# Gadersd/stable-diffusion-xl-burn

Hardware: NVIDIA H100
Metric: unet_sampler_steps_per_sec_1024x1024_bs1 (higher is better)
Workload: dtype f16

## Files before the change

### stable-diffusion-xl-burn_b200/csrc/common.cuh

```cuda
#pragma once
#include <cuda_fp16.h>
#include <cuda_runtime.h>
#include <stdint.h>
#include <stdio.h>

namespace sdxl {

__device__ __forceinline__ uint32_t smem_u32(const void* p) {
  return static_cast<uint32_t>(__cvta_generic_to_shared(p));
}
__device__ __forceinline__ float warp_sum(float v) {
#pragma unroll
  for (int o = 16; o > 0; o >>= 1) v += __shfl_xor_sync(0xffffffffu, v, o);
  return v;
}
__device__ __forceinline__ float warp_max(float v) {
#pragma unroll
  for (int o = 16; o > 0; o >>= 1) v = fmaxf(v, __shfl_xor_sync(0xffffffffu, v, o));
  return v;
}
__device__ __forceinline__ float silu_f(float x) { return x / (1.0f + __expf(-x)); }
__device__ __forceinline__ float erf_as(float x) {
  const float ax = fabsf(x);
  float t;
// ... 37 lines not shown
__device__ __forceinline__ void mbar_arrive(uint64_t* bar) {
  asm volatile("mbarrier.arrive.shared::cta.b64 _, [%0];" ::"r"(smem_u32(bar)) : "memory");
}
__device__ __forceinline__ bool mbar_try_wait(uint64_t* bar, uint32_t parity) {
  uint32_t ok;
  asm volatile(
      "{\n\t"
      ".reg .pred p;\n\t"
      "mbarrier.try_wait.parity.shared::cta.b64 p, [%1], %2;\n\t"
      "selp.u32 %0, 1, 0, p;\n\t"
      "}"
      : "=r"(ok)
      : "r"(smem_u32(bar)), "r"(parity)
      : "memory");
  return ok != 0;
}
__device__ __forceinline__ void mbar_wait(uint64_t* bar, uint32_t parity) {
  if (mbar_try_wait(bar, parity)) return;
  const uint64_t t0 = globaltimer_ns();
  while (!mbar_try_wait(bar, parity)) {
    if (globaltimer_ns() - t0 > 4000000000ull) {
      printf("sdxl_b200: mbarrier wait timeout (block %d,%d,%d thread %d)\n", blockIdx.x, blockIdx.y,
             blockIdx.z, threadIdx.x);
      __trap();
    }
  }
}
__device__ __forceinline__ void mbar_wait_nocall(uint64_t* bar, uint32_t parity) {
  if (mbar_try_wait(bar, parity)) return;
  const uint64_t t0 = globaltimer_ns();
  while (!mbar_try_wait(bar, parity))
    if (globaltimer_ns() - t0 > 4000000000ull) __trap();
}
__device__ __forceinline__ void fence_proxy_async_smem() {
  asm volatile("fence.proxy.async.shared::cta;" ::: "memory");
}

__device__ __forceinline__ void tma_prefetch_desc(const void* tmap) {
  asm volatile("prefetch.tensormap [%0];" ::"l"(reinterpret_cast<uint64_t>(tmap)) : "memory");
}
__device__ __forceinline__ void tma_load_2d(void* dst, const void* tmap, uint64_t* bar, int c0, int c1) {
  asm volatile(
      "cp.async.bulk.tensor.2d.shared::cluster.global.mbarrier::complete_tx::bytes [%0], [%1, {%3, %4}], [%2];"
      ::"r"(smem_u32(dst)), "l"(reinterpret_cast<uint64_t>(tmap)), "r"(smem_u32(bar)), "r"(c0), "r"(c1)
      : "memory");
}
__device__ __forceinline__ void tma_load_3d(void* dst, const void* tmap, uint64_t* bar, int c0, int c1,
                                            int c2) {
  asm volatile(
      "cp.async.bulk.tensor.3d.shared::cluster.global.mbarrier::complete_tx::bytes [%0], [%1, {%3, %4, %5}], [%2];"
      ::"r"(smem_u32(dst)), "l"(reinterpret_cast<uint64_t>(tmap)), "r"(smem_u32(bar)), "r"(c0), "r"(c1),
      "r"(c2)
      : "memory");
}
__device__ __forceinline__ void tma_load_4d(void* dst, const void* tmap, uint64_t* bar, int c0, int c1,
                                            int c2, int c3) {
  asm volatile(
      "cp.async.bulk.tensor.4d.shared::cluster.global.mbarrier::complete_tx::bytes [%0], [%1, {%3, %4, %5, %6}], [%2];"
      ::"r"(smem_u32(dst)), "l"(reinterpret_cast<uint64_t>(tmap)), "r"(smem_u32(bar)), "r"(c0), "r"(c1),
      "r"(c2), "r"(c3)
      : "memory");
}

__device__ __forceinline__ void wg_fence() { asm volatile("wgmma.fence.sync.aligned;" ::: "memory"); }
__device__ __forceinline__ void wg_commit() { asm volatile("wgmma.commit_group.sync.aligned;" ::: "memory"); }
template <int N>
__device__ __forceinline__ void wg_wait() {
  asm volatile("wgmma.wait_group.sync.aligned %0;" ::"n"(N) : "memory");
}
__device__ __forceinline__ uint64_t wg_desc_sw128(uint32_t saddr) {
  const uint32_t lo = ((saddr >> 4) & 0x3FFFu) | (1u << 16);
  const uint32_t hi = 64u  | (1u << 30) ;
  return (static_cast<uint64_t>(hi) << 32) | lo;
}
__device__ __forceinline__ void wgmma_ss_n160(float (&d)[80], uint64_t da, uint64_t db, int scale_d) {
  asm volatile(
      "{\n\t.reg .pred p;\n\tsetp.ne.b32 p, %82, 0;\n\t"
// ... 28 lines not shown
```

### stable-diffusion-xl-burn_b200/csrc/engine_core.h

```cpp
#pragma once
#include "../../include/sdxl_b200.h"
#include "kernels.h"

#include <math.h>
#include <nvtx3/nvToolsExt.h>
#include <stdarg.h>
#include <stdio.h>
#include <stdlib.h>
#include <string.h>

#include <map>
#include <memory>
#include <string>
#include <type_traits>
#include <vector>

using namespace sdxl;

struct sdxl_ctx {
  int device = 0;
  cudaStream_t stream = nullptr;
  bool own_stream = false;
  int num_sms = 132;
  std::string err;
// ... 686 lines not shown
  for (size_t i = 0; i < n && !r; ++i) {
    r = exec_op(c, P->ops[i]);
    if (!r && cudaEventRecord(ev[i + 1], c->stream) != cudaSuccess) r = -2;
  }
  cudaError_t se = cudaStreamSynchronize(c->stream);
  ms.assign(n, 0.f);
  if (!r && se == cudaSuccess)
    for (size_t i = 0; i < n; ++i) cudaEventElapsedTime(&ms[i], ev[i], ev[i + 1]);
  for (auto& e : ev) cudaEventDestroy(e);
  if (se != cudaSuccess) return fail(c, (int)se, "profile run failed: %s", cudaGetErrorString(se));
  return r;
}

static int profile_plan_impl(sdxl_ctx* c, Plan* P, double* ms_by_kind, double* flops_by_kind, int* launches_by_kind) {
  std::vector<float> ms;
  const int r = time_plan_ops(c, P, ms);
  for (int k = 0; k < SDXL_PROFILE_KINDS; ++k) { ms_by_kind[k] = 0; flops_by_kind[k] = 0; launches_by_kind[k] = 0; }
  if (r) return r;
  for (size_t i = 0; i < ms.size(); ++i) {
    const int k = (int)P->ops[i].kind;
    if (k < 0 || k >= SDXL_PROFILE_KINDS) continue;
    ms_by_kind[k] += ms[i];
    flops_by_kind[k] += P->ops[i].flops;
    launches_by_kind[k] += (P->ops[i].kind == OP_GN) ? 2 : 1;
  }
  return 0;
}

static int profile_dump_impl(sdxl_ctx* c, Plan* P, const char* path) {
  std::vector<float> ms;
  if (int r = time_plan_ops(c, P, ms)) return r;
  FILE* f = fopen(path, "w");
  if (!f) return fail(c, -3, "cannot open %s", path);
  fprintf(f, "op,kind,us,gflop,tflops,M_tiles,N,BN,Kblocks,T,S,heads\n");
  for (size_t i = 0; i < ms.size(); ++i) {
    const Op& o = P->ops[i];
    int mt = 0, N = 0, BN = 0, kb = 0, T = 0, S = 0, H = 0;
    if (o.kind == OP_IGEMM) {
      mt = o.ig.tilesW * o.ig.tilesH * o.ig.tilesB; N = o.ig.N; BN = o.ig.BN;
      for (int s2 = 0; s2 < o.ig.nseg; ++s2) kb += o.ig.seg[s2].nkb;
    } else if (o.kind == OP_ATTN) { T = o.at.T; S = o.at.S; H = o.at.n_head; }
    fprintf(f, "%zu,%s,%.2f,%.3f,%.1f,%d,%d,%d,%d,%d,%d,%d\n", i, kOpNames[o.kind], ms[i] * 1e3, o.flops * 1e-9,
            ms[i] > 0 ? o.flops / (ms[i] * 1e-3) * 1e-12 : 0.0, mt, N, BN, kb, T, S, H);
  }
  fclose(f);
  return 0;
}

struct TmpBufs {
  std::vector<void*> p;
  cudaStream_t st;
  int fill = debug_fill_byte();
  explicit TmpBufs(cudaStream_t s) : st(s) {}
  template <typename T>
  T* get(size_t bytes) {
    void* d = nullptr;
    if (cudaMallocAsync(&d, bytes ? bytes : 16, st) != cudaSuccess) return nullptr;
    p.push_back(d);
    if (fill >= 0) debug_fill((T*)d, bytes / sizeof(T), st, fill);
    return (T*)d;
  }
  ~TmpBufs() { for (void* d : p) cudaFreeAsync(d, st); }
};

static int adapters_apply(sdxl_ctx* c, AdapterState& S, int n, const sdxl_adapter* ad) {
  if (n < 0 || n > SDXL_MAX_ADAPTERS) return fail(c, 4600, "set_adapters: n = %d outside [0, %d]", n, SDXL_MAX_ADAPTERS);
  if (n > 0 && !ad) return fail(c, 4601, "set_adapters: null adapter array");
  TmpBufs tmp(c->stream);
  std::map<std::string, std::vector<LoraTerm>> terms;
  for (int a = 0; a < n; ++a) {
    PackView pv;
    std::vector<uint8_t> table;
    if (!ad[a].pack) return fail(c, 4602, "set_adapters: adapter %d has a null pack", a);
    int r = parse_pack(c, ad[a].pack, ad[a].bytes, ad[a].pack_on_device, pv, table);
    if (r) { c->err = "adapter " + std::to_string(a) + ": " + c->err; return r; }
    if (ad[a].pack_on_device) {
// ... 113 lines not shown
```

### stable-diffusion-xl-burn_b200/csrc/igemm.cu

```cuda
#include "common.cuh"
#include "kernels.h"

#include <stdio.h>
#include <stdlib.h>

namespace sdxl {

static constexpr int kTileM = 128;
static constexpr int kBlockK = 64;
static constexpr int kABytes = kTileM * kBlockK * 2;
static constexpr int kConsumerWarps = 8;
static constexpr int kThreads = 128 + kConsumerWarps * 32;

__device__ __forceinline__ size_t out_pixel(const IgemmParams& p, int tb, int th, int tw, int r, bool& ok, int& bb) {
  const int wt = r % p.Wt, ht = (r / p.Wt) % p.Ht, bt = r / (p.Wt * p.Ht);
  bb = tb * p.Bt + bt;
  const int hh = th * p.Ht + ht, ww = tw * p.Wt + wt;
  ok = (bb < p.Bn) && (hh < p.H) && (ww < p.W);
  return ok ? ((size_t)bb * p.H + hh) * (size_t)p.opix_row + (size_t)ww * p.opix_w + p.opix_off : 0;
}

__device__ __forceinline__ void store2(const IgemmParams& p, size_t off, float x0, float x1, bool two, bool vec) {
  if (p.out_f32) {
    float* o = reinterpret_cast<float*>(p.out) + off;
// ... 34 lines not shown
          bv[jj] = rv[jj] = make_float2(0.f, 0.f);
          if (n >= p.N) continue;
          if (bias) bv[jj] = (two && vec) ? __ldg(reinterpret_cast<const float2*>(bias + n)) : make_float2(bias[n], two ? bias[n + 1] : 0.f);
          if (res) rv[jj] = (two && vec) ? *reinterpret_cast<const float2*>(res + n) : make_float2(res[n], two ? res[n + 1] : 0.f);
        }
#pragma unroll
        for (int jj = 0; jj < JC; ++jj) {
          const int j = j0 + jj, n = n0 + 8 * j + cq;
          if (n >= p.N) continue;
          float x0 = acc[4 * j + 2 * h], x1 = acc[4 * j + 2 * h + 1];
          if (bias) { x0 += bv[jj].x; x1 += bv[jj].y; }
          if (res) { x0 += rv[jj].x; x1 += rv[jj].y; }
          store2(p, pix * p.ldo + n, x0, x1, n + 1 < p.N, vec);
        }
      }
    } else {
      constexpr int hb = BN / 2;
#pragma unroll
      for (int j = 0; j < hb / 8; ++j) {
        const int c = 8 * j + cq;
        float x0 = acc[4 * j + 2 * h], x1 = acc[4 * j + 2 * h + 1];
        float y0 = acc[4 * (j + hb / 8) + 2 * h], y1 = acc[4 * (j + hb / 8) + 2 * h + 1];
        if (p.bias != nullptr) {
          x0 += __ldg(p.bias + n0 + c); x1 += __ldg(p.bias + n0 + c + 1);
          y0 += __ldg(p.bias + n0 + hb + c); y1 += __ldg(p.bias + n0 + hb + c + 1);
        }
        reinterpret_cast<__half2*>(reinterpret_cast<__half*>(p.out) + pix * p.ldo + nt * hb + c)[0] =
            __floats2half2_rn(x0 * gelu_erf_f(y0), x1 * gelu_erf_f(y1));
      }
    }
  }
}

template <int BN>
__global__ void __launch_bounds__(kThreads, 1) igemm_kernel(const __grid_constant__ IgemmParams p) {
  constexpr int NC = BN == 160 ? 160 : BN >= 128 ? 128 : 64;
  constexpr int NCH = BN / NC;
  extern __shared__ __align__(1024) uint8_t smem_raw[];
  uint8_t* smem = reinterpret_cast<uint8_t*>((reinterpret_cast<uintptr_t>(smem_raw) + 1023) & ~uintptr_t(1023));
  const int nst = p.nstages;
  constexpr uint32_t stage_bytes = kABytes + BN * 128;
  uint64_t* full_bar = reinterpret_cast<uint64_t*>(smem + (size_t)nst * stage_bytes);
  uint64_t* empty_bar = full_bar + nst;

  const int warp = threadIdx.x >> 5, lane = threadIdx.x & 31;
  const int m_tiles = p.tilesW * p.tilesH * p.tilesB;
  const int num_tiles = m_tiles * p.tilesN;
  int total_kb = 0;
  for (int s = 0; s < p.nseg; ++s) total_kb += p.seg[s].nkb;

  if (threadIdx.x == 0) {
    for (int i = 0; i < nst; ++i) { mbar_init(&full_bar[i], 1); mbar_init(&empty_bar[i], kConsumerWarps); }
    fence_barrier_init();
    tma_prefetch_desc(&p.tmA0);
    tma_prefetch_desc(&p.tmA1);
    tma_prefetch_desc(&p.tmB);
  }
  __syncthreads();
  griddep_wait();
  griddep_launch_dependents();

  if (warp < 4) {
    setmaxnreg_dec<40>();
    if (warp != 0 || lane != 0) return;
    uint32_t stage = 0, phase = 0;
    for (int st = blockIdx.x; st < num_tiles; st += gridDim.x) {
      const int mt = st % m_tiles, nt = st / m_tiles;
      const int tw = mt % p.tilesW, th = (mt / p.tilesW) % p.tilesH, tb = mt / (p.tilesW * p.tilesH);
      const int w0 = tw * p.Wt, h0 = th * p.Ht, b0 = tb * p.Bt, n0 = nt * BN;
      int kcol = 0;
      for (int s = 0; s < p.nseg; ++s) {
        const IgemmSeg sg = p.seg[s];
        const void* mapA = sg.map ? (const void*)&p.tmA1 : (const void*)&p.tmA0;
        for (int j = 0; j < sg.nkb; ++j, kcol += kBlockK) {
          mbar_wait_nocall(&empty_bar[stage], phase ^ 1);
          uint8_t* dst = smem + stage * stage_bytes;
          mbar_expect_tx(&full_bar[stage], stage_bytes);
          tma_load_4d(dst, mapA, &full_bar[stage], j * kBlockK, w0 + sg.dw, h0 + sg.dh, b0 + sg.db);
          tma_load_2d(dst + kABytes, &p.tmB, &full_bar[stage], kcol, n0);
          if (++stage == (uint32_t)nst) { stage = 0; phase ^= 1; }
        }
      }
    }
    return;
  }

  setmaxnreg_inc<232>();
  const int wg = (warp >> 2) - 1;
  const int r0 = wg * 64 + (warp & 3) * 16 + (lane >> 2);
  const uint32_t smem_base = smem_u32(smem);
  uint32_t stage = 0, phase = 0;
  float acc[BN / 2];
  for (int st = blockIdx.x; st < num_tiles; st += gridDim.x) {
    const int mt = st % m_tiles, nt = st / m_tiles;
    uint32_t prev = 0;
    for (int kb = 0; kb < total_kb; ++kb) {
      mbar_wait_nocall(&full_bar[stage], phase);
      wg_fence();
      const uint32_t a = smem_base + stage * stage_bytes + (uint32_t)wg * (64 * 128);
      const uint32_t b = smem_base + stage * stage_bytes + kABytes;
#pragma unroll
      for (int k = 0; k < kBlockK / 16; ++k) {
        const uint64_t da = wg_desc_sw128(a + 32 * k);
#pragma unroll
        for (int c = 0; c < NCH; ++c) {
          const uint64_t db = wg_desc_sw128(b + c * NC * 128 + 32 * k);
          if constexpr (NC == 160) wgmma_ss_n160(*reinterpret_cast<float(*)[80]>(acc), da, db, (kb | k) != 0);
          else if constexpr (NC == 128) wgmma_ss_n128(*reinterpret_cast<float(*)[64]>(acc + 64 * c), da, db, (kb | k) != 0);
          else wgmma_ss_n64(*reinterpret_cast<float(*)[32]>(acc + 32 * c), da, db, (kb | k) != 0);
        }
      }
      wg_commit();
      if (kb > 0) {
        wg_wait<1>();
        if (lane == 0) mbar_arrive(&empty_bar[prev]);
      }
      prev = stage;
      if (++stage == (uint32_t)nst) { stage = 0; phase ^= 1; }
    }
    wg_wait<0>();
    if (lane == 0 && total_kb > 0) mbar_arrive(&empty_bar[prev]);
    const int tw = mt % p.tilesW, th = (mt / p.tilesW) % p.tilesH, tb = mt / (p.tilesW * p.tilesH);
    epilogue<BN>(p, acc, tb, th, tw, nt, r0, lane);
  }
}

typedef CUresult (*PFN_encodeTiled)(CUtensorMap*, CUtensorMapDataType, cuuint32_t, void*, const cuuint64_t*,
                                    const cuuint64_t*, const cuuint32_t*, const cuuint32_t*,
                                    CUtensorMapInterleave, CUtensorMapSwizzle, CUtensorMapL2promotion,
                                    CUtensorMapFloatOOBfill);
static PFN_encodeTiled get_encode() {
  static PFN_encodeTiled fn = nullptr;
  if (!fn) {
    void* f = nullptr;
    cudaDriverEntryPointQueryResult qres;
    if (cudaGetDriverEntryPoint("cuTensorMapEncodeTiled", &f, cudaEnableDefault, &qres) != cudaSuccess ||
        qres != cudaDriverEntryPointSuccess)
      return nullptr;
    fn = reinterpret_cast<PFN_encodeTiled>(f);
  }
  return fn;
}

static int encode(CUtensorMap* tm, const void* base, int rank, const uint64_t* dims, const uint64_t* strides_bytes,
                  const uint32_t* box, CUtensorMapDataType dtype = CU_TENSOR_MAP_DATA_TYPE_FLOAT16,
                  CUtensorMapSwizzle swz = CU_TENSOR_MAP_SWIZZLE_128B) {
  PFN_encodeTiled fn = get_encode();
  if (!fn) return 1001;
  cuuint64_t gd[5];
  cuuint64_t gs[5];
  cuuint32_t bx[5], es[5];
  for (int i = 0; i < rank; ++i) {
    gd[i] = dims[i];
    bx[i] = box[i];
    es[i] = 1;
    if (i > 0) gs[i - 1] = strides_bytes[i - 1];
// ... 29 lines not shown
  uint64_t str[2] = {(uint64_t)pitch * 2, (uint64_t)rows_per_batch * pitch * 2};
  uint32_t box[3] = {64, 128, 1};
  return encode(tm, base, 3, dims, str, box);
}

void igemm_pick_box(int W, int H, int* Wt, int* Ht, int* Bt) {
  int wt = 1;
  while (wt * 2 <= W && wt * 2 <= 128) wt *= 2;
  int ht = 1;
  while (ht * 2 <= H && wt * ht * 2 <= 128) ht *= 2;
  *Wt = wt;
  *Ht = ht;
  *Bt = 128 / (wt * ht);
}

int igemm_pick_bn(int m_tiles, int N, int num_sms, bool geglu) {
  (void)geglu;
  double best = 1e30;
  int best_bn = 0;
  for (int bn : {256, 160, 128, 64}) {
    if (N % bn) continue;
    const long tiles = (long)m_tiles * (N / bn);
    const long waves = (tiles + num_sms - 1) / num_sms;
    const double cost = (double)waves * (bn + 48.0);
    if (cost < best) {
      best = cost;
      best_bn = bn;
    }
  }
  if (!best_bn) best_bn = N <= 64 ? 64 : N <= 128 ? 128 : 256;
  return best_bn;
}

struct IgemmDev { bool attr = false; int num_sms = 0; };
static IgemmDev g_igemm_dev[64];
static IgemmDev* igemm_dev() {
  int dev = 0;
  if (cudaGetDevice(&dev) != cudaSuccess || dev < 0 || dev >= 64) return nullptr;
  IgemmDev& D = g_igemm_dev[dev];
  if (!D.num_sms) {
    cudaDeviceGetAttribute(&D.num_sms, cudaDevAttrMultiProcessorCount, dev);
    if (D.num_sms <= 0) D.num_sms = 132;
  }
  return &D;
}
static int device_sms() {
  IgemmDev* D = igemm_dev();
  return D ? D->num_sms : 132;
}

static constexpr int kMaxSmem = 227 * 1024;
static size_t igemm_smem_bytes(int nst, int BN) { return (size_t)nst * (kABytes + BN * 128) + 1024  + 2 * nst * 8; }

int igemm_configure(IgemmParams& p, const IgemmOperands& o, int outW, int outH, int outB, int mode, int geglu_bn) {
  igemm_pick_box(outW, outH, &p.Wt, &p.Ht, &p.Bt);
  p.W = outW; p.H = outH; p.Bn = outB;
  p.opix_row = outW; p.opix_w = 1; p.opix_off = 0;
  p.tilesW = (outW + p.Wt - 1) / p.Wt;
  p.tilesH = (outH + p.Ht - 1) / p.Ht;
  p.tilesB = (outB + p.Bt - 1) / p.Bt;
  const int m_tiles = p.tilesW * p.tilesH * p.tilesB;
  p.N = o.N;
  p.mode = mode;
  p.BN = (mode == IGEMM_GEGLU) ? geglu_bn : igemm_pick_bn(m_tiles, o.N, device_sms(), false);
  if (p.BN != 64 && p.BN != 128 && p.BN != 160 && p.BN != 256) return 1010;
  p.tilesN = (mode == IGEMM_GEGLU) ? (o.N / p.BN) : ((o.N + p.BN - 1) / p.BN);
  int r = make_tmap_act(&p.tmA0, o.a0, o.a0Bn, o.a0H, o.a0W, o.a0C, o.a0pitch, p.Wt, p.Ht, p.Bt);
  if (!r && o.a1) r = make_tmap_act(&p.tmA1, o.a1, o.a1Bn, o.a1H, o.a1W, o.a1C, o.a1pitch, p.Wt, p.Ht, p.Bt);
  if (!r && !o.a1) p.tmA1 = p.tmA0;
  if (!r) r = make_tmap_wgt(&p.tmB, o.w, o.N, o.Ktot, p.BN);
  if (r) return r;
  const int stage_bytes = kABytes + p.BN * 128;
  int nst = (kMaxSmem - 1024 - 256) / stage_bytes;
  if (nst > 8) nst = 8;
  p.nstages = nst;
  return 0;
}

int igemm_launch(cudaStream_t st, IgemmParams& p) {
  if (p.res != nullptr && p.ldr != p.ldo) return 1003;
  if ((unsigned long long)p.Bn * p.H * (unsigned long long)p.opix_row * (unsigned long long)p.ldo >= (1ull << 32)) return 1004;
  if (p.nstages < 2) return 1011;
  const size_t smem = igemm_smem_bytes(p.nstages, p.BN);
  if (smem > (size_t)kMaxSmem) return 1011;
  IgemmDev* D = igemm_dev();
  if (!D) return 1009;
  if (!D->attr) {
    cudaError_t e = cudaFuncSetAttribute(igemm_kernel<64>, cudaFuncAttributeMaxDynamicSharedMemorySize, kMaxSmem);
    if (e == cudaSuccess) e = cudaFuncSetAttribute(igemm_kernel<128>, cudaFuncAttributeMaxDynamicSharedMemorySize, kMaxSmem);
    if (e == cudaSuccess) e = cudaFuncSetAttribute(igemm_kernel<160>, cudaFuncAttributeMaxDynamicSharedMemorySize, kMaxSmem);
    if (e == cudaSuccess) e = cudaFuncSetAttribute(igemm_kernel<256>, cudaFuncAttributeMaxDynamicSharedMemorySize, kMaxSmem);
    if (e != cudaSuccess) return (int)e;
    D->attr = true;
  }
  const long tiles = (long)p.tilesW * p.tilesH * p.tilesB * p.tilesN;
  const dim3 grid((unsigned)(tiles < D->num_sms ? (tiles > 0 ? tiles : 1) : D->num_sms));
  switch (p.BN) {
    case 64: return launch_kernel(igemm_kernel<64>, grid, dim3(kThreads), smem, st, true, p);
    case 128: return launch_kernel(igemm_kernel<128>, grid, dim3(kThreads), smem, st, true, p);
    case 160: return launch_kernel(igemm_kernel<160>, grid, dim3(kThreads), smem, st, true, p);
    case 256: return launch_kernel(igemm_kernel<256>, grid, dim3(kThreads), smem, st, true, p);
    default: return 1010;
  }
}

}
```

### stable-diffusion-xl-burn_b200/csrc/kernels.h

```cpp
#pragma once
#include <cuda.h>
#include <cuda_fp16.h>
#include <cuda_runtime.h>
#include <stdint.h>

namespace sdxl {

bool pdl_enabled();
template <typename... KArgs, typename... Args>
inline int launch_kernel(void (*kernel)(KArgs...), dim3 grid, dim3 block, size_t smem, cudaStream_t st, bool pdl,
                         Args&&... args) {
  cudaLaunchConfig_t cfg{};
  cfg.gridDim = grid;
  cfg.blockDim = block;
  cfg.dynamicSmemBytes = smem;
  cfg.stream = st;
  cudaLaunchAttribute attr[1];
  attr[0].id = cudaLaunchAttributeProgrammaticStreamSerialization;
  attr[0].val.programmaticStreamSerializationAllowed = 1;
  cfg.attrs = attr;
  cfg.numAttrs = (pdl && pdl_enabled()) ? 1 : 0;
  return (int)cudaLaunchKernelEx(&cfg, kernel, static_cast<KArgs>(args)...);
}
template <typename... KArgs, typename... Args>
// ... 34 lines not shown
    if (e != cudaSuccess) return (int)e;
    done[dev] = true;
  }
  return 0;
}

constexpr int IGEMM_MAX_SEG = 20;
struct IgemmSeg {
  int16_t map;
  int16_t dw, dh;
  int16_t db;
  int32_t nkb;
};
enum IgemmMode : int { IGEMM_LINEAR = 0, IGEMM_GEGLU = 1 };
struct alignas(64) IgemmParams {
  CUtensorMap tmA0, tmA1, tmB;
  IgemmSeg seg[IGEMM_MAX_SEG];
  int nseg;
  int Wt, Ht, Bt;
  int W, H, Bn;
  int tilesW, tilesH, tilesB, tilesN;
  int N;
  int BN;
  int nstages;
  int mode;
  void* out;
  int out_f32;
  int ldo;
  const float* bias;
  int bias_bstride;
  const float* res;
  int ldr;
  int opix_row, opix_w, opix_off;
};
int make_tmap_act(CUtensorMap* tm, const __half* base, int Bn, int H, int W, int C, int pitch, int Wt,
                  int Ht, int Bt);
int make_tmap_wgt(CUtensorMap* tm, const __half* base, int N, int K, int BN);
void igemm_pick_box(int W, int H, int* Wt, int* Ht, int* Bt);
struct IgemmOperands {
  const __half* a0; int a0Bn, a0H, a0W, a0C, a0pitch;
  const __half* a1; int a1Bn, a1H, a1W, a1C, a1pitch;
  const __half* w; int N, Ktot;
};
int igemm_configure(IgemmParams& p, const IgemmOperands& o, int outW, int outH, int outB, int mode, int geglu_bn);
int igemm_launch(cudaStream_t st, IgemmParams& p);
int igemm_pick_bn(int m_tiles, int N, int num_sms, bool geglu);

constexpr int ATTN_MAX_SRC = 8;
struct AttnIpSource {
  CUtensorMap tm;
  int S, k_col0, v_col0;
  const float* scale;
  const float* mask;
};
struct AttnParams {
  CUtensorMap tmQ, tmK, tmV;
  int T, S, n_head, B;
  int q_col0, k_col0, v_col0;
  __half* out;
  int ldo;
  float scale_log2e;
  CUtensorMap tmKip, tmVip;
  int S_ip;
  int k_ip_col0, v_ip_col0;
  const float* ip_scale;
  int n_src;
  const float* ip_mask;
  AttnIpSource ip_src[ATTN_MAX_SRC - 1];
};
int make_tmap_rows(CUtensorMap* tm, const __half* base, int rows_per_batch, int nbatch, int cols, int pitch);
int attention_launch(cudaStream_t st, const AttnParams& p);
int ip_mask_resize_launch(cudaStream_t st, const float* mask, int H, int W, int mh, int mw, int T, float* out);

struct GnParams {
  const float* x1; int C1;
  const float* x2; int C2;
  int B, HW, n_group;
  const float* gamma; const float* beta;
// ... 121 lines not shown
```

### stable-diffusion-xl-burn_b200/csrc/testing.cu

```cuda
#include "kernels.h"
#include "schedule.h"

#define SDXL_TEST_API extern "C" __attribute__((visibility("default")))

using namespace sdxl;

SDXL_TEST_API int sdxl_test_igemm(void* stream, const void* a0, int a0Bn, int a0H, int a0W, int a0C, int a0pitch, const void* a1,
                                  int a1Bn, int a1H, int a1W, int a1C, int a1pitch, const void* w, int N, int Ktot, int outW,
                                  int outH, int outB, int mode, int geglu_bn, const int* segs, int nseg, void* out, int out_f32,
                                  int ldo, const float* bias, int bias_bstride, const float* res, int ldr, int opix_row,
                                  int opix_w, int opix_off) {
  if (nseg < 1 || nseg > IGEMM_MAX_SEG) return 5002;
  IgemmParams p{};
  p.nseg = nseg;
  for (int i = 0; i < nseg; ++i)
    p.seg[i] = {(int16_t)segs[5 * i], (int16_t)segs[5 * i + 1], (int16_t)segs[5 * i + 2], (int16_t)segs[5 * i + 3], segs[5 * i + 4]};
  p.out = out; p.out_f32 = out_f32; p.ldo = ldo;
  p.bias = bias; p.bias_bstride = bias_bstride;
  p.res = res; p.ldr = ldr;
  const IgemmOperands o{(const __half*)a0, a0Bn, a0H, a0W, a0C, a0pitch, (const __half*)a1, a1Bn, a1H, a1W, a1C, a1pitch,
                        (const __half*)w, N, Ktot};
  if (int r = igemm_configure(p, o, outW, outH, outB, mode, geglu_bn)) return r;
  if (opix_row) { p.opix_row = opix_row; p.opix_w = opix_w; p.opix_off = opix_off; }
  return igemm_launch((cudaStream_t)stream, p);
}

SDXL_TEST_API int sdxl_test_attention(void* stream, const void* q, int q_pitch, int q_col0, const void* kv, int kv_pitch, int k_col0,
                                      int v_col0, int B, int T, int S, int n_head, void* out, int ldo, const void* kip,
                                      int kip_pitch, int k_ip_col0, int v_ip_col0, int S_ip, const float* ip_scale) {
  AttnParams p{};
  p.T = T; p.S = S; p.n_head = n_head; p.B = B;
  p.q_col0 = q_col0; p.k_col0 = k_col0; p.v_col0 = v_col0;
  p.out = (__half*)out; p.ldo = ldo;
  p.scale_log2e = (float)(1.4426950408889634 / 8.0);
  int r = make_tmap_rows(&p.tmQ, (const __half*)q, T, B, q_pitch, q_pitch);
  if (!r) r = make_tmap_rows(&p.tmK, (const __half*)kv, S, B, kv_pitch, kv_pitch);
  if (r) return r;
  p.tmV = p.tmK;
  if (kip) {
    p.S_ip = S_ip; p.k_ip_col0 = k_ip_col0; p.v_ip_col0 = v_ip_col0; p.ip_scale = ip_scale; p.n_src = 1;
    if ((r = make_tmap_rows(&p.tmKip, (const __half*)kip, S_ip, B, kip_pitch, kip_pitch))) return r;
    p.tmVip = p.tmKip;
  }
  return attention_launch((cudaStream_t)stream, p);
}

SDXL_TEST_API int sdxl_test_attention_multi(void* stream, const void* q, int q_pitch, int q_col0, const void* kv, int kv_pitch, int k_col0,
                                            int v_col0, int B, int T, int S, int n_head, void* out, int ldo, int n_src,
                                            const void* const* src_kv, const int* src_info, const float* const* scales,
                                            const float* const* masks) {
  if (n_src < 1 || n_src > ATTN_MAX_SRC) return 5003;
  AttnParams p{};
  p.T = T; p.S = S; p.n_head = n_head; p.B = B;
  p.q_col0 = q_col0; p.k_col0 = k_col0; p.v_col0 = v_col0;
  p.out = (__half*)out; p.ldo = ldo;
  p.scale_log2e = (float)(1.4426950408889634 / 8.0);
// ... 227 lines not shown
```

### stable-diffusion-xl-burn_b200/sdxl_b200/_testing.py

```python
from __future__ import annotations

import ctypes as C
import os
from typing import Optional, Sequence

import torch

from ._lib import SdxlError, SdxlLibraryMissing

HERE = os.path.dirname(os.path.abspath(__file__))
LIB_PATH = os.path.join(HERE, "libsdxl_b200_testing.so")

P, I, F, L, Z = C.c_void_p, C.c_int, C.c_float, C.c_long, C.c_size_t
PROTOTYPES = {
    "sdxl_test_igemm": (I, [P, P, I, I, I, I, I, P, I, I, I, I, I, P, I, I, I, I, I, I, I, P, I, P, I, I, P, I, P, I, I, I, I]),
    "sdxl_test_attention": (I, [P, P, I, I, P, I, I, I, I, I, I, I, P, I, P, I, I, I, I, P]),
    "sdxl_test_attention_multi": (I, [P, P, I, I, P, I, I, I, I, I, I, I, P, I, I, P, P, P, P]),
    "sdxl_test_ip_mask_resize": (I, [P, P, I, I, I, I, I, P]),
    "sdxl_test_attention_small": (I, [P, P, I, I, P, P, I, I, I, I, I, I, I, P, I, P, I, I]),
    "sdxl_test_perceiver_ln": (I, [P, P, P, I, I, I, I, P, P, P, P, F, P, P]),
    "sdxl_test_gn_scratch_floats": (C.c_size_t, [I, I]),
    "sdxl_test_gn_scratch_init": (I, [P, P, I, I]),
    "sdxl_test_gn": (I, [P, P, I, P, I, I, I, I, P, P, F, I, P, P, P, P]),
    "sdxl_test_gemv": (I, [P, P, I, I, I, P, I, P, P, I, I, I, I, P, I]),
    "sdxl_test_conv_in": (I, [P, P, I, I, I, I, I, I, P, P, I, P, P, I]),
    "sdxl_test_conv_in_cat": (I, [P, P, I, I, I, I, P, I, I, I, I, P, P, I, P]),
    "sdxl_test_pag_identity": (I, [P, P, I, C.c_long, P]),
    "sdxl_test_cfg_pag_ddim": (I, [P, P, I, I, I, I, I, F, F, F, F, F, F, P]),
    "sdxl_test_freeu_twiddles": (None, [I, I, P]),
    "sdxl_test_freeu": (I, [P, P, I, P, I, I, I, I, P, P, P]),
    "sdxl_test_repack_upconv": (I, [P, P, I, I, P, I]),
    "sdxl_test_repack_conv": (I, [P, P, I, I, I, I, P, I, I, I]),
    "sdxl_test_transpose_linear": (I, [P, P, I, I, P, I, I, I]),
    "sdxl_test_bias_to_f32": (I, [P, P, I, P, I, I]),
    "sdxl_test_lora_merge": (I, [P, I, I, I, I, P, P, P, P, P, P, I, C.c_size_t, I, I, I, I, P]),
    "sdxl_test_lora_upconv_merge": (I, [P, P, P, I, I, P, I]),
    "sdxl_test_softmax_rows": (I, [P, P, Z, I, I, F, P, Z]),
    "sdxl_test_transpose_f16": (I, [P, P, Z, I, I, P, Z]),
    "sdxl_test_post_quant": (I, [P, P, I, I, I, P, P, F, P]),
    "sdxl_test_quant_out": (I, [P, P, I, I, I, L, P, P, F, P]),
    "sdxl_test_image_u8": (I, [P, P, L, I, P]),
    "sdxl_test_image_from_u8": (I, [P, P, I, L, P]),
    "sdxl_test_embed_tokens": (I, [P, P, I, I, I, I, P, P, P, P]),
    "sdxl_test_patchify": (I, [P, P, I, I, I, I, P]),
    "sdxl_test_vision_embed_ln": (I, [P, P, P, P, I, I, I, P, P, F, P]),
    "sdxl_test_mlp_act": (I, [P, P, Z, I, P]),
    "sdxl_test_ln_gather_f32": (I, [P, P, P, I, I, I, P, P, F, P]),
    "sdxl_test_pixel_unshuffle": (I, [P, P, I, I, I, I, P]),
# ... 18 lines not shown
    "sdxl_test_timestep_embedding_f32": (I, [P, P, I, I, F, P]),
}
_lib = None


def load() -> C.CDLL:
    global _lib
    if _lib is None:
        if not os.path.exists(LIB_PATH):
            raise SdxlLibraryMissing(f"{LIB_PATH} not found: build it with `python stable-diffusion-xl-burn_b200/build.py`")
        lib = C.CDLL(LIB_PATH)
        for name, (res, args) in PROTOTYPES.items():
            fn = getattr(lib, name)
            fn.restype = res
            fn.argtypes = args
        _lib = lib
    return _lib


def _p(t: Optional[torch.Tensor]):
    if t is None:
        return None
    assert t.is_cuda and t.is_contiguous(), "kernel operands are contiguous CUDA tensors"
    return t.data_ptr()


def _call(name: str, *args) -> None:
    lib = load()
    rc = getattr(lib, name)(torch.cuda.current_stream().cuda_stream, *args)
    if rc != 0:
        raise SdxlError(f"{name} failed ({rc})")


def igemm(a0: torch.Tensor, a0_shape: Sequence[int], w: torch.Tensor, N: int, Ktot: int, out_whb: Sequence[int],
          segs: Sequence[Sequence[int]], out: torch.Tensor, ldo: int, *, a1: Optional[torch.Tensor] = None,
          a1_shape: Sequence[int] = (0, 0, 0, 0), bias: Optional[torch.Tensor] = None, bias_bstride: int = 0,
          res: Optional[torch.Tensor] = None, ldr: int = 0, mode: int = 0, geglu_bn: int = 0,
          opix: Optional[Sequence[int]] = None) -> None:
    seg = (C.c_int * (5 * len(segs)))(*[int(v) for s in segs for v in s])
    o = opix or (0, 0, 0)
    _call("sdxl_test_igemm", _p(a0), *a0_shape, a0_shape[3], _p(a1), *a1_shape, a1_shape[3], _p(w), N, Ktot, *out_whb, mode,
          geglu_bn, seg, len(segs), _p(out), int(out.dtype == torch.float32), ldo, _p(bias), bias_bstride, _p(res), ldr, *o)


def attention(q: torch.Tensor, q_pitch: int, q_col0: int, kv: torch.Tensor, kv_pitch: int, k_col0: int, v_col0: int,
              B: int, T: int, S: int, n_head: int, out: torch.Tensor, ldo: int, kip: Optional[torch.Tensor] = None,
              kip_pitch: int = 0, k_ip_col0: int = 0, v_ip_col0: int = 0, S_ip: int = 0,
              ip_scale: Optional[torch.Tensor] = None) -> None:
    _call("sdxl_test_attention", _p(q), q_pitch, q_col0, _p(kv), kv_pitch, k_col0, v_col0, B, T, S, n_head, _p(out), ldo,
          _p(kip), kip_pitch, k_ip_col0, v_ip_col0, S_ip, _p(ip_scale))


def attention_multi(q: torch.Tensor, q_pitch: int, q_col0: int, kv: torch.Tensor, kv_pitch: int, k_col0: int, v_col0: int,
                    B: int, T: int, S: int, n_head: int, out: torch.Tensor, ldo: int, sources: Sequence[tuple]) -> None:
    n = len(sources)
    kvs = (C.c_void_p * n)(*[_p(s[0]) for s in sources])
    info = (C.c_int * (4 * n))(*[int(v) for s in sources for v in (s[1], s[2], s[3], s[4])])
    scales = (C.c_void_p * n)(*[_p(s[5]) for s in sources])
    masks = (C.c_void_p * n)(*[_p(s[6]) for s in sources])
    _call("sdxl_test_attention_multi", _p(q), q_pitch, q_col0, _p(kv), kv_pitch, k_col0, v_col0, B, T, S, n_head, _p(out), ldo, n,
          kvs, info, scales, masks)


def ip_mask_resize(mask: torch.Tensor, mh: int, mw: int, T: int) -> torch.Tensor:
    out = torch.empty(T, device=mask.device, dtype=torch.float32)
    _call("sdxl_test_ip_mask_resize", _p(mask), mask.shape[0], mask.shape[1], mh, mw, T, _p(out))
    return out


def attention_small(q, q_pitch, q_col0, k, v, kv_pitch, k_col0, v_col0, B, T, S, n_head, mask, causal, out, ldo,
                    head_dim) -> None:
    _call("sdxl_test_attention_small", _p(q), q_pitch, q_col0, _p(k), _p(v), kv_pitch, k_col0, v_col0, B, T, S, n_head,
          _p(mask), int(causal), _p(out), ldo, head_dim)


# ... 202 lines not shown
```

Before: 27.34.

## Add 2-CTA cluster mode with TMA multicast of weight tiles in igemm

Adds a cluster-of-2 variant of the implicit-GEMM kernel in which paired CTAs along M each load half of the shared B (weight) tile and multicast it to both CTAs. Empty barriers now count arrivals from both CTAs so a stage is refilled only once both consumers have released it. Auto policy enables clusters only when tiles fit in one wave and M tiles are even, aiming to halve weight-load traffic for small-grid GEMMs. Risks include extra cross-CTA synchronization, cluster scheduling limits, and a drain loop at producer exit.

```diff
diff --git a/stable-diffusion-xl-burn_b200/csrc/common.cuh b/stable-diffusion-xl-burn_b200/csrc/common.cuh
--- a/stable-diffusion-xl-burn_b200/csrc/common.cuh
+++ b/stable-diffusion-xl-burn_b200/csrc/common.cuh
@@ -93,6 +93,24 @@
   while (!mbar_try_wait(bar, parity))
     if (globaltimer_ns() - t0 > 4000000000ull) __trap();
 }
+__device__ __forceinline__ void mbar_arrive_cluster(uint64_t* bar, uint32_t cta) {
+  asm volatile(
+      "{\n\t.reg .b32 ra;\n\t"
+      "mapa.shared::cluster.u32 ra, %0, %1;\n\t"
+      "mbarrier.arrive.shared::cluster.b64 _, [ra];\n\t}"
+      ::"r"(smem_u32(bar)), "r"(cta)
+      : "memory");
+}
+
+__device__ __forceinline__ uint32_t cluster_ctarank() {
+  uint32_t r;
+  asm volatile("mov.u32 %0, %%cluster_ctarank;" : "=r"(r));
+  return r;
+}
+__device__ __forceinline__ void cluster_sync_relaxed() {
+  asm volatile("barrier.cluster.arrive.relaxed;\n\tbarrier.cluster.wait;" ::: "memory");
+}
+
 __device__ __forceinline__ void fence_proxy_async_smem() {
   asm volatile("fence.proxy.async.shared::cta;" ::: "memory");
 }
@@ -104,6 +122,12 @@
   asm volatile(
       "cp.async.bulk.tensor.2d.shared::cluster.global.mbarrier::complete_tx::bytes [%0], [%1, {%3, %4}], [%2];"
       ::"r"(smem_u32(dst)), "l"(reinterpret_cast<uint64_t>(tmap)), "r"(smem_u32(bar)), "r"(c0), "r"(c1)
+      : "memory");
+}
+__device__ __forceinline__ void tma_load_2d_multicast(void* dst, const void* tmap, uint64_t* bar, int c0, int c1, uint16_t cta_mask) {
+  asm volatile(
+      "cp.async.bulk.tensor.2d.shared::cluster.global.mbarrier::complete_tx::bytes.multicast::cluster [%0], [%1, {%3, %4}], [%2], %5;"
+      ::"r"(smem_u32(dst)), "l"(reinterpret_cast<uint64_t>(tmap)), "r"(smem_u32(bar)), "r"(c0), "r"(c1), "h"(cta_mask)
       : "memory");
 }
 __device__ __forceinline__ void tma_load_3d(void* dst, const void* tmap, uint64_t* bar, int c0, int c1,
diff --git a/stable-diffusion-xl-burn_b200/csrc/engine_core.h b/stable-diffusion-xl-burn_b200/csrc/engine_core.h
--- a/stable-diffusion-xl-burn_b200/csrc/engine_core.h
+++ b/stable-diffusion-xl-burn_b200/csrc/engine_core.h
@@ -742,16 +742,16 @@
   if (int r = time_plan_ops(c, P, ms)) return r;
   FILE* f = fopen(path, "w");
   if (!f) return fail(c, -3, "cannot open %s", path);
-  fprintf(f, "op,kind,us,gflop,tflops,M_tiles,N,BN,Kblocks,T,S,heads\n");
+  fprintf(f, "op,kind,us,gflop,tflops,M_tiles,N,BN,Kblocks,T,S,heads,cluster\n");
   for (size_t i = 0; i < ms.size(); ++i) {
     const Op& o = P->ops[i];
-    int mt = 0, N = 0, BN = 0, kb = 0, T = 0, S = 0, H = 0;
+    int mt = 0, N = 0, BN = 0, kb = 0, T = 0, S = 0, H = 0, cl = 0;
     if (o.kind == OP_IGEMM) {
-      mt = o.ig.tilesW * o.ig.tilesH * o.ig.tilesB; N = o.ig.N; BN = o.ig.BN;
+      mt = o.ig.tilesW * o.ig.tilesH * o.ig.tilesB; N = o.ig.N; BN = o.ig.BN; cl = o.ig.cluster;
       for (int s2 = 0; s2 < o.ig.nseg; ++s2) kb += o.ig.seg[s2].nkb;
     } else if (o.kind == OP_ATTN) { T = o.at.T; S = o.at.S; H = o.at.n_head; }
-    fprintf(f, "%zu,%s,%.2f,%.3f,%.1f,%d,%d,%d,%d,%d,%d,%d\n", i, kOpNames[o.kind], ms[i] * 1e3, o.flops * 1e-9,
-            ms[i] > 0 ? o.flops / (ms[i] * 1e-3) * 1e-12 : 0.0, mt, N, BN, kb, T, S, H);
+    fprintf(f, "%zu,%s,%.2f,%.3f,%.1f,%d,%d,%d,%d,%d,%d,%d,%d\n", i, kOpNames[o.kind], ms[i] * 1e3, o.flops * 1e-9,
+            ms[i] > 0 ? o.flops / (ms[i] * 1e-3) * 1e-12 : 0.0, mt, N, BN, kb, T, S, H, cl);
   }
   fclose(f);
   return 0;
diff --git a/stable-diffusion-xl-burn_b200/csrc/igemm.cu b/stable-diffusion-xl-burn_b200/csrc/igemm.cu
--- a/stable-diffusion-xl-burn_b200/csrc/igemm.cu
+++ b/stable-diffusion-xl-burn_b200/csrc/igemm.cu
@@ -90,8 +90,9 @@
   }
 }
 
-template <int BN>
+template <int BN, int CL>
 __global__ void __launch_bounds__(kThreads, 1) igemm_kernel(const __grid_constant__ IgemmParams p) {
+  static_assert(CL == 1 || CL == 2, "clusters of 1 or 2 CTAs along M");
   constexpr int NC = BN == 160 ? 160 : BN >= 128 ? 128 : 64;
   constexpr int NCH = BN / NC;
   extern __shared__ __align__(1024) uint8_t smem_raw[];
@@ -108,19 +109,21 @@
   for (int s = 0; s < p.nseg; ++s) total_kb += p.seg[s].nkb;
 
   if (threadIdx.x == 0) {
-    for (int i = 0; i < nst; ++i) { mbar_init(&full_bar[i], 1); mbar_init(&empty_bar[i], kConsumerWarps); }
+    for (int i = 0; i < nst; ++i) { mbar_init(&full_bar[i], 1); mbar_init(&empty_bar[i], CL * kConsumerWarps); }
     fence_barrier_init();
     tma_prefetch_desc(&p.tmA0);
     tma_prefetch_desc(&p.tmA1);
     tma_prefetch_desc(&p.tmB);
   }
-  __syncthreads();
+  if constexpr (CL > 1) cluster_sync_relaxed();
+  else __syncthreads();
   griddep_wait();
   griddep_launch_dependents();
 
   if (warp < 4) {
     setmaxnreg_dec<40>();
     if (warp != 0 || lane != 0) return;
+    const int rank = CL > 1 ? (int)cluster_ctarank() : 0;
     uint32_t stage = 0, phase = 0;
     for (int st = blockIdx.x; st < num_tiles; st += gridDim.x) {
       const int mt = st % m_tiles, nt = st / m_tiles;
@@ -135,11 +138,19 @@
           uint8_t* dst = smem + stage * stage_bytes;
           mbar_expect_tx(&full_bar[stage], stage_bytes);
           tma_load_4d(dst, mapA, &full_bar[stage], j * kBlockK, w0 + sg.dw, h0 + sg.dh, b0 + sg.db);
-          tma_load_2d(dst + kABytes, &p.tmB, &full_bar[stage], kcol, n0);
+          if constexpr (CL > 1)
+            tma_load_2d_multicast(dst + kABytes + rank * (BN / 2) * 128, &p.tmB, &full_bar[stage], kcol, n0 + rank * (BN / 2), 0x3);
+          else
+            tma_load_2d(dst + kABytes, &p.tmB, &full_bar[stage], kcol, n0);
           if (++stage == (uint32_t)nst) { stage = 0; phase ^= 1; }
         }
       }
     }
+    if constexpr (CL > 1)
+      for (int i = 0; i < nst; ++i) {
+        mbar_wait_nocall(&empty_bar[stage], phase ^ 1);
+        if (++stage == (uint32_t)nst) { stage = 0; phase ^= 1; }
+      }
     return;
   }
 
@@ -171,15 +182,22 @@
       wg_commit();
       if (kb > 0) {
         wg_wait<1>();
-        if (lane == 0) mbar_arrive(&empty_bar[prev]);
+        if (lane == 0) {
+          mbar_arrive(&empty_bar[prev]);
+          if constexpr (CL > 1) mbar_arrive_cluster(&empty_bar[prev], cluster_ctarank() ^ 1);
+        }
       }
       prev = stage;
       if (++stage == (uint32_t)nst) { stage = 0; phase ^= 1; }
     }
     wg_wait<0>();
-    if (lane == 0 && total_kb > 0) mbar_arrive(&empty_bar[prev]);
+    if (lane == 0 && total_kb > 0) {
+      mbar_arrive(&empty_bar[prev]);
+      if constexpr (CL > 1) mbar_arrive_cluster(&empty_bar[prev], cluster_ctarank() ^ 1);
+    }
     const int tw = mt % p.tilesW, th = (mt / p.tilesW) % p.tilesH, tb = mt / (p.tilesW * p.tilesH);
     epilogue<BN>(p, acc, tb, th, tw, nt, r0, lane);
+    if constexpr (CL > 1) break;
   }
 }
 
@@ -275,7 +293,7 @@
   return best_bn;
 }
 
-struct IgemmDev { bool attr = false; int num_sms = 0; };
+struct IgemmDev { bool attr = false; int num_sms = 0; int max_clusters[4] = {-1, -1, -1, -1}; };
 static IgemmDev g_igemm_dev[64];
 static IgemmDev* igemm_dev() {
   int dev = 0;
@@ -294,8 +312,76 @@
 
 static constexpr int kMaxSmem = 227 * 1024;
 static size_t igemm_smem_bytes(int nst, int BN) { return (size_t)nst * (kABytes + BN * 128) + 1024  + 2 * nst * 8; }
-
-int igemm_configure(IgemmParams& p, const IgemmOperands& o, int outW, int outH, int outB, int mode, int geglu_bn) {
+static int igemm_nstages(int BN) {
+  const int nst = (kMaxSmem - 1024 - 256) / (kABytes + BN * 128);
+  return nst > 8 ? 8 : nst;
+}
+static int bn_index(int BN) { return BN == 64 ? 0 : BN == 128 ? 1 : BN == 160 ? 2 : 3; }
+
+template <int CL>
+static void* igemm_kernel_ptr(int BN) {
+  switch (BN) {
+    case 64: return (void*)igemm_kernel<64, CL>;
+    case 128: return (void*)igemm_kernel<128, CL>;
+    case 160: return (void*)igemm_kernel<160, CL>;
+    case 256: return (void*)igemm_kernel<256, CL>;
+    default: return nullptr;
+  }
+}
+
+static int igemm_dev_attr(IgemmDev* D) {
+  if (D->attr) return 0;
+  for (int bn : {64, 128, 160, 256})
+    for (void* k : {igemm_kernel_ptr<1>(bn), igemm_kernel_ptr<2>(bn)}) {
+      cudaError_t e = cudaFuncSetAttribute(k, cudaFuncAttributeMaxDynamicSharedMemorySize, kMaxSmem);
+      if (e != cudaSuccess) return (int)e;
+    }
+  D->attr = true;
+  return 0;
+}
+
+int igemm_max_clusters(int BN) {
+  IgemmDev* D = igemm_dev();
+  void* k = igemm_kernel_ptr<2>(BN);
+  if (!D || !k || igemm_dev_attr(D)) return 0;
+  int& n = D->max_clusters[bn_index(BN)];
+  if (n < 0) {
+    cudaLaunchConfig_t cfg{};
+    cfg.gridDim = dim3(2);
+    cfg.blockDim = dim3(kThreads);
+    cfg.dynamicSmemBytes = igemm_smem_bytes(igemm_nstages(BN), BN);
+    cudaLaunchAttribute a[1];
+    a[0].id = cudaLaunchAttributeClusterDimension;
+    a[0].val.clusterDim.x = 2;
+    a[0].val.clusterDim.y = 1;
+    a[0].val.clusterDim.z = 1;
+    cfg.attrs = a;
+    cfg.numAttrs = 1;
+    if (cudaOccupancyMaxActiveClusters(&n, k, &cfg) != cudaSuccess) {
+      cudaGetLastError();
+      n = 0;
+    }
+  }
+  return n;
+}
+
+static bool igemm_cluster_disabled() {
+  static const bool off = getenv("SDXL_B200_NO_IGEMM_CLUSTER") != nullptr;
+  return off;
+}
+
+static int igemm_pick_cluster(const IgemmParams& p, int policy) {
+  const long m_tiles = (long)p.tilesW * p.tilesH * p.tilesB;
+  if (policy == IGEMM_CLUSTER_OFF || (policy == IGEMM_CLUSTER_AUTO && igemm_cluster_disabled())) return 1;
+  if (m_tiles % 2 != 0 || (p.tilesN - 1) * p.BN + p.BN / 2 >= p.N) return 1;
+  const int mc = igemm_max_clusters(p.BN);
+  if (mc <= 0) return 1;
+  if (policy == IGEMM_CLUSTER_ON) return 2;
+  const long tiles = m_tiles * p.tilesN;
+  return tiles <= device_sms() && tiles / 2 <= mc ? 2 : 1;
+}
+
+int igemm_configure(IgemmParams& p, const IgemmOperands& o, int outW, int outH, int outB, int mode, int geglu_bn, int cluster) {
   igemm_pick_box(outW, outH, &p.Wt, &p.Ht, &p.Bt);
   p.W = outW; p.H = outH; p.Bn = outB;
   p.opix_row = outW; p.opix_w = 1; p.opix_off = 0;
@@ -308,16 +394,13 @@
   p.BN = (mode == IGEMM_GEGLU) ? geglu_bn : igemm_pick_bn(m_tiles, o.N, device_sms(), false);
   if (p.BN != 64 && p.BN != 128 && p.BN != 160 && p.BN != 256) return 1010;
   p.tilesN = (mode == IGEMM_GEGLU) ? (o.N / p.BN) : ((o.N + p.BN - 1) / p.BN);
+  p.nstages = igemm_nstages(p.BN);
+  p.cluster = igemm_pick_cluster(p, cluster);
   int r = make_tmap_act(&p.tmA0, o.a0, o.a0Bn, o.a0H, o.a0W, o.a0C, o.a0pitch, p.Wt, p.Ht, p.Bt);
   if (!r && o.a1) r = make_tmap_act(&p.tmA1, o.a1, o.a1Bn, o.a1H, o.a1W, o.a1C, o.a1pitch, p.Wt, p.Ht, p.Bt);
   if (!r && !o.a1) p.tmA1 = p.tmA0;
-  if (!r) r = make_tmap_wgt(&p.tmB, o.w, o.N, o.Ktot, p.BN);
-  if (r) return r;
-  const int stage_bytes = kABytes + p.BN * 128;
-  int nst = (kMaxSmem - 1024 - 256) / stage_bytes;
-  if (nst > 8) nst = 8;
-  p.nstages = nst;
-  return 0;
+  if (!r) r = make_tmap_wgt(&p.tmB, o.w, o.N, o.Ktot, p.BN / p.cluster);
+  return r;
 }
 
 int igemm_launch(cudaStream_t st, IgemmParams& p) {
@@ -328,21 +411,25 @@
   if (smem > (size_t)kMaxSmem) return 1011;
   IgemmDev* D = igemm_dev();
   if (!D) return 1009;
-  if (!D->attr) {
-    cudaError_t e = cudaFuncSetAttribute(igemm_kernel<64>, cudaFuncAttributeMaxDynamicSharedMemorySize, kMaxSmem);
-    if (e == cudaSuccess) e = cudaFuncSetAttribute(igemm_kernel<128>, cudaFuncAttributeMaxDynamicSharedMemorySize, kMaxSmem);
-    if (e == cudaSuccess) e = cudaFuncSetAttribute(igemm_kernel<160>, cudaFuncAttributeMaxDynamicSharedMemorySize, kMaxSmem);
-    if (e == cudaSuccess) e = cudaFuncSetAttribute(igemm_kernel<256>, cudaFuncAttributeMaxDynamicSharedMemorySize, kMaxSmem);
-    if (e != cudaSuccess) return (int)e;
-    D->attr = true;
-  }
+  if (int e = igemm_dev_attr(D)) return e;
   const long tiles = (long)p.tilesW * p.tilesH * p.tilesB * p.tilesN;
+  if (p.cluster == 2) {
+    const dim3 grid((unsigned)tiles);
+    switch (p.BN) {
+      case 64: return launch_kernel_cluster(igemm_kernel<64, 2>, grid, dim3(kThreads), smem, st, true, 2, p);
+      case 128: return launch_kernel_cluster(igemm_kernel<128, 2>, grid, dim3(kThreads), smem, st, true, 2, p);
+      case 160: return launch_kernel_cluster(igemm_kernel<160, 2>, grid, dim3(kThreads), smem, st, true, 2, p);
+      case 256: return launch_kernel_cluster(igemm_kernel<256, 2>, grid, dim3(kThreads), smem, st, true, 2, p);
+      default: return 1010;
+    }
+  }
+  if (p.cluster != 1) return 1012;
   const dim3 grid((unsigned)(tiles < D->num_sms ? (tiles > 0 ? tiles : 1) : D->num_sms));
   switch (p.BN) {
-    case 64: return launch_kernel(igemm_kernel<64>, grid, dim3(kThreads), smem, st, true, p);
-    case 128: return launch_kernel(igemm_kernel<128>, grid, dim3(kThreads), smem, st, true, p);
-    case 160: return launch_kernel(igemm_kernel<160>, grid, dim3(kThreads), smem, st, true, p);
-    case 256: return launch_kernel(igemm_kernel<256>, grid, dim3(kThreads), smem, st, true, p);
+    case 64: return launch_kernel(igemm_kernel<64, 1>, grid, dim3(kThreads), smem, st, true, p);
+    case 128: return launch_kernel(igemm_kernel<128, 1>, grid, dim3(kThreads), smem, st, true, p);
+    case 160: return launch_kernel(igemm_kernel<160, 1>, grid, dim3(kThreads), smem, st, true, p);
+    case 256: return launch_kernel(igemm_kernel<256, 1>, grid, dim3(kThreads), smem, st, true, p);
     default: return 1010;
   }
 }
diff --git a/stable-diffusion-xl-burn_b200/csrc/kernels.h b/stable-diffusion-xl-burn_b200/csrc/kernels.h
--- a/stable-diffusion-xl-burn_b200/csrc/kernels.h
+++ b/stable-diffusion-xl-burn_b200/csrc/kernels.h
@@ -90,6 +90,7 @@
   const float* res;
   int ldr;
   int opix_row, opix_w, opix_off;
+  int cluster;
 };
 int make_tmap_act(CUtensorMap* tm, const __half* base, int Bn, int H, int W, int C, int pitch, int Wt,
                   int Ht, int Bt);
@@ -100,8 +101,11 @@
   const __half* a1; int a1Bn, a1H, a1W, a1C, a1pitch;
   const __half* w; int N, Ktot;
 };
-int igemm_configure(IgemmParams& p, const IgemmOperands& o, int outW, int outH, int outB, int mode, int geglu_bn);
+enum IgemmCluster : int { IGEMM_CLUSTER_AUTO = -1, IGEMM_CLUSTER_OFF = 0, IGEMM_CLUSTER_ON = 1 };
+int igemm_configure(IgemmParams& p, const IgemmOperands& o, int outW, int outH, int outB, int mode, int geglu_bn,
+                    int cluster = IGEMM_CLUSTER_AUTO);
 int igemm_launch(cudaStream_t st, IgemmParams& p);
+int igemm_max_clusters(int BN);
 int igemm_pick_bn(int m_tiles, int N, int num_sms, bool geglu);
 
 constexpr int ATTN_MAX_SRC = 8;
diff --git a/stable-diffusion-xl-burn_b200/csrc/testing.cu b/stable-diffusion-xl-burn_b200/csrc/testing.cu
--- a/stable-diffusion-xl-burn_b200/csrc/testing.cu
+++ b/stable-diffusion-xl-burn_b200/csrc/testing.cu
@@ -9,7 +9,7 @@
                                   int a1Bn, int a1H, int a1W, int a1C, int a1pitch, const void* w, int N, int Ktot, int outW,
                                   int outH, int outB, int mode, int geglu_bn, const int* segs, int nseg, void* out, int out_f32,
                                   int ldo, const float* bias, int bias_bstride, const float* res, int ldr, int opix_row,
-                                  int opix_w, int opix_off) {
+                                  int opix_w, int opix_off, int cluster, int* info) {
   if (nseg < 1 || nseg > IGEMM_MAX_SEG) return 5002;
   IgemmParams p{};
   p.nseg = nseg;
@@ -20,8 +20,12 @@
   p.res = res; p.ldr = ldr;
   const IgemmOperands o{(const __half*)a0, a0Bn, a0H, a0W, a0C, a0pitch, (const __half*)a1, a1Bn, a1H, a1W, a1C, a1pitch,
                         (const __half*)w, N, Ktot};
-  if (int r = igemm_configure(p, o, outW, outH, outB, mode, geglu_bn)) return r;
+  if (int r = igemm_configure(p, o, outW, outH, outB, mode, geglu_bn, cluster)) return r;
   if (opix_row) { p.opix_row = opix_row; p.opix_w = opix_w; p.opix_off = opix_off; }
+  if (info) {
+    info[0] = p.BN; info[1] = p.tilesW * p.tilesH * p.tilesB * p.tilesN; info[2] = p.nstages;
+    info[3] = p.cluster; info[4] = igemm_max_clusters(p.BN);
+  }
   return igemm_launch((cudaStream_t)stream, p);
 }
 
diff --git a/stable-diffusion-xl-burn_b200/sdxl_b200/_testing.py b/stable-diffusion-xl-burn_b200/sdxl_b200/_testing.py
--- a/stable-diffusion-xl-burn_b200/sdxl_b200/_testing.py
+++ b/stable-diffusion-xl-burn_b200/sdxl_b200/_testing.py
@@ -2,7 +2,7 @@
 
 import ctypes as C
 import os
-from typing import Optional, Sequence
+from typing import Dict, Optional, Sequence
 
 import torch
 
@@ -13,7 +13,7 @@
 
 P, I, F, L, Z = C.c_void_p, C.c_int, C.c_float, C.c_long, C.c_size_t
 PROTOTYPES = {
-    "sdxl_test_igemm": (I, [P, P, I, I, I, I, I, P, I, I, I, I, I, P, I, I, I, I, I, I, I, P, I, P, I, I, P, I, P, I, I, I, I]),
+    "sdxl_test_igemm": (I, [P, P, I, I, I, I, I, P, I, I, I, I, I, P, I, I, I, I, I, I, I, P, I, P, I, I, P, I, P, I, I, I, I, I, P]),
     "sdxl_test_attention": (I, [P, P, I, I, P, I, I, I, I, I, I, I, P, I, P, I, I, I, I, P]),
     "sdxl_test_attention_multi": (I, [P, P, I, I, P, I, I, I, I, I, I, I, P, I, I, P, P, P, P]),
     "sdxl_test_ip_mask_resize": (I, [P, P, I, I, I, I, I, P]),
@@ -98,15 +98,21 @@
         raise SdxlError(f"{name} failed ({rc})")
 
 
+CLUSTER_AUTO, CLUSTER_OFF, CLUSTER_ON = -1, 0, 1
+
+
 def igemm(a0: torch.Tensor, a0_shape: Sequence[int], w: torch.Tensor, N: int, Ktot: int, out_whb: Sequence[int],
           segs: Sequence[Sequence[int]], out: torch.Tensor, ldo: int, *, a1: Optional[torch.Tensor] = None,
           a1_shape: Sequence[int] = (0, 0, 0, 0), bias: Optional[torch.Tensor] = None, bias_bstride: int = 0,
           res: Optional[torch.Tensor] = None, ldr: int = 0, mode: int = 0, geglu_bn: int = 0,
-          opix: Optional[Sequence[int]] = None) -> None:
+          opix: Optional[Sequence[int]] = None, cluster: int = CLUSTER_AUTO) -> Dict[str, int]:
     seg = (C.c_int * (5 * len(segs)))(*[int(v) for s in segs for v in s])
     o = opix or (0, 0, 0)
+    info = (C.c_int * 5)()
     _call("sdxl_test_igemm", _p(a0), *a0_shape, a0_shape[3], _p(a1), *a1_shape, a1_shape[3], _p(w), N, Ktot, *out_whb, mode,
-          geglu_bn, seg, len(segs), _p(out), int(out.dtype == torch.float32), ldo, _p(bias), bias_bstride, _p(res), ldr, *o)
+          geglu_bn, seg, len(segs), _p(out), int(out.dtype == torch.float32), ldo, _p(bias), bias_bstride, _p(res), ldr, *o,
+          cluster, info)
+    return dict(zip(("BN", "tiles", "stages", "cluster", "max_clusters"), info))
 
 
 def attention(q: torch.Tensor, q_pitch: int, q_col0: int, kv: torch.Tensor, kv_pitch: int, k_col0: int, v_col0: int,
```

Result: no change. 27.48 (median of 6 runs) (+0.5%).
